# timmeinhardt/trackformer

Measured on AMD Instinct MI355X. Metric: frames/sec, TrackFormer-Deformable inference (ResNet-50, 1333x800, 300 object + 100 track queries, bs 1 per GPU); roofline = ms_deform_attn HBM GB/s, higher is better.
Workload: dtype f32 (dense layers as the fp16 split product on MFMA: two fp16 pieces per activation, three per weight scaled per output channel -- 22 + 1 significand bits per operand, the one dropped product < 2^-22 --, three terms, f32 accumulate)

## Files before the change

include/tf_fused.h:

```cpp
#ifndef TF_FUSED_H_
#define TF_FUSED_H_

#include <stdint.h>

#ifdef __cplusplus
extern "C" {
#endif

int tf_bias_act_f32(float *x, const float *bias, const float *residual, int64_t n, int C, int relu,
                    void *stream);

int tf_add_layernorm_f32(const float *x, const float *res, const float *gamma, const float *beta,
                         float *out, int64_t rows, int C, float eps, void *stream);

int tf_box_refine_f32(const float *delta, const float *ref, float *out, int64_t rows, int ref_dim, float eps, void *stream);

int tf_postprocess_pack_f32(const float *logits, const float *boxes, float *out, int64_t Q, int C, float img_h, float img_w,
                            int clip, void *stream);

int tf_groupnorm_nhwc_f32(const float *x, const float *gamma, const float *beta, float *out, double *workspace, int N,
                          int HW, int C, int G, float eps, int64_t x_image_stride, int64_t out_image_stride, void *stream);
int tf_groupnorm_stats_nhwc_f32(const float *x, double *workspace, int N, int HW, int C, int G, int64_t x_image_stride, void *stream);
int tf_groupnorm_relu_nhwc_f32(const float *x, const float *gamma, const float *beta, float *out, double *workspace, int N,
                               int HW, int C, int G, float eps, int64_t x_image_stride, int64_t out_image_stride, void *stream);
// ... 43 lines not shown
int tf_linear_packed_f32(const float *x, const void *w_packed, const float *bias, const float *residual, float *y, int64_t M, int K,
                         int N, int relu, int terms, void *stream);

int64_t tf_linear_grad_stats_workspace_bytes(int64_t M, int C, int role, int with_colsum);
int tf_linear_grad_stats_f32(const float *a, float *scale2, float *colsum, void *workspace, int64_t workspace_bytes, int64_t M, int C,
                             int role, int terms, void *stream);
int64_t tf_linear_wgrad_workspace_bytes(int64_t M, int K, int N);
int tf_linear_wgrad_split_f32(const float *dy, const float *x, const float *dy_scale2, const float *x_scale2, float *dw, void *workspace,
                              int64_t workspace_bytes, int64_t M, int K, int N, int terms, void *stream);
int tf_linear_dgrad_packed_f32(const float *dy, const float *dy_scale2, const void *wt_packed, float *dx, int64_t M, int K, int N,
                               int terms, void *stream);

int tf_conv_packed_f32(const float *x, const void *w_packed, const float *bias, const float *residual, float *y, float *workspace,
                       int ksplit, int nimg, int hin, int win, int cin, int cout, int ks, int stride, int relu, int terms,
                       void *stream);

int tf_linear_res_ln_f32(const float *x, const void *w_packed, const float *bias, const float *residual, const float *ln_weight,
                         const float *ln_bias, float ln_eps, float *y, int64_t M, int K, int N, int terms, void *stream);

int tf_ffn_fused_f32(const float *x, const void *w1_packed, const float *b1, const void *w2_packed, const float *b2,
                     const float *residual, const float *ln_weight, const float *ln_bias, float ln_eps, float *y, int64_t M,
                     int d_model, int d_ffn, int terms, void *stream);

int tf_mha_core_f32(const float *q, const float *k, const float *v, float *out, const unsigned char *key_mask,
                    int N, int Lq, int Lk, int H, int D, int ldq, int ldk, int ldv, int ldo, float scale,
                    void *stream);

int tf_nms_host_f32(const float *boxes, const float *scores, int n, float iou_threshold, int64_t *keep, int *n_keep);

#ifdef __cplusplus
}
#endif
#endif
```

trackformer_amd/_cabi.py:

```python
import ctypes
import os

_PKG_DIR = os.path.dirname(os.path.abspath(__file__))
LIB_PATH = os.environ.get("TF_MSDA_LIB") or os.path.join(_PKG_DIR, "lib", "libtf_msda.so")

EXPORTED_SYMBOLS = (
    "tf_msda_abi_version",
    "tf_msda_strerror",
    "tf_msda_last_hip_error",
    "tf_msda_last_kernel",
    "tf_msda_set_tiled",
    "tf_msda_set_option",
    "tf_msda_debug_trace_buffer",
    "tf_msda_forward_fused_f32",
    "tf_msda_forward_f32",
    "tf_msda_forward_f64",
    "tf_msda_forward_f32_dshapes",
    "tf_msda_forward_f64_dshapes",
    "tf_msda_backward_f32",
    "tf_msda_backward_f64",
    "tf_msda_backward_f32_dshapes",
    "tf_msda_backward_f64_dshapes",
    "tf_msda_backward_det_workspace_bytes",
    "tf_msda_backward_det_f32",
# ... 16 lines not shown
    "tf_mask_label_map_f32",
    "tf_conv3x3_merge_packed_f32",
    "tf_groupnorm_stats_nhwc_f32",
    "tf_groupnorm_relu_conv3x3_c1_nhwc_f32",
    "tf_bias_relu_maxpool_f32",
    "tf_stem_conv7x7_f32",
    "tf_linear_split_f32",
    "tf_linear_split_res_f32",
    "tf_conv3x3_split_f32",
    "tf_conv3x3_splitk_f32",
    "tf_conv1x1_strided_split_f32",
    "tf_conv1x1_splitk_f32",
    "tf_linear_packed_bytes",
    "tf_linear_pack_weight_f32",
    "tf_linear_packed_f32",
    "tf_linear_grad_stats_workspace_bytes",
    "tf_linear_grad_stats_f32",
    "tf_linear_wgrad_workspace_bytes",
    "tf_linear_wgrad_split_f32",
    "tf_linear_dgrad_packed_f32",
    "tf_linear_split_add_f32",
    "tf_ffn_fused_f32",
    "tf_linear_res_ln_f32",
    "tf_conv_packed_f32",
    "tf_mha_core_f32",
    "tf_nms_host_f32",
)

ABI_VERSION = 6

_lib = None


class MSDAError(RuntimeError):
    """Raised when libtf_msda.so reports a non-zero status."""


def lib():
    global _lib
    if _lib is not None:
        return _lib
    if not os.path.exists(LIB_PATH):
        raise RuntimeError(
            "trackformer_amd: native library %s not found. Build it with "
            "`python -m trackformer_amd.build` (needs hipcc); there is no CPU fallback." % LIB_PATH)
    import torch
    L = ctypes.CDLL(LIB_PATH)
    vp, ci = ctypes.c_void_p, ctypes.c_int
    L.tf_msda_abi_version.restype = ci
    L.tf_msda_abi_version.argtypes = []
    L.tf_msda_strerror.restype = ctypes.c_char_p
    L.tf_msda_strerror.argtypes = [ci]
    L.tf_msda_last_hip_error.restype = ci
    L.tf_msda_last_hip_error.argtypes = []
# ... 58 lines not shown
    for fn in (L.tf_groupnorm_nhwc_f32, L.tf_groupnorm_relu_nhwc_f32):
        fn.restype = ci
        fn.argtypes = [vp, vp, vp, vp, vp, ci, ci, ci, ci, ctypes.c_float, ctypes.c_int64, ctypes.c_int64, vp]
    L.tf_linear_split_f32.restype = ci
    L.tf_linear_split_f32.argtypes = [vp, vp, vp, vp, vp, vp, vp, ctypes.c_int64, ci, ci, ci, vp]
    L.tf_linear_split_res_f32.restype = ci
    L.tf_linear_split_res_f32.argtypes = [vp, vp, vp, vp, vp, vp, vp, vp, ctypes.c_int64, ci, ci, ci, vp]
    L.tf_conv3x3_splitk_f32.restype = ci
    L.tf_conv3x3_splitk_f32.argtypes = [vp, vp, vp, vp, vp, vp, vp, vp, ci, ci, ci, ci, ci, ci, ci, ci, vp]
    L.tf_conv3x3_split_f32.restype = ci
    L.tf_conv3x3_split_f32.argtypes = [vp, vp, vp, vp, vp, vp, vp] + [ci] * 7 + [vp]
    L.tf_conv1x1_splitk_f32.restype = ci
    L.tf_conv1x1_splitk_f32.argtypes = [vp, vp, vp, vp, vp, vp, vp, vp, ci, ci, ci, ci, ci, ci, ci, ci, vp]
    L.tf_conv1x1_strided_split_f32.restype = ci
    L.tf_conv1x1_strided_split_f32.argtypes = [vp, vp, vp, vp, vp, vp, vp] + [ci] * 7 + [vp]
    L.tf_linear_packed_bytes.restype = ctypes.c_int64
    L.tf_linear_packed_bytes.argtypes = [ci, ci, ci]
    L.tf_linear_pack_weight_f32.restype = ci
    L.tf_linear_pack_weight_f32.argtypes = [vp, vp, ci, ci, ci, vp]
    L.tf_linear_res_ln_f32.restype = ci
    L.tf_linear_res_ln_f32.argtypes = [vp, vp, vp, vp, vp, vp, ctypes.c_float, vp, ctypes.c_int64, ci, ci, ci, vp]
    L.tf_ffn_fused_f32.restype = ci
    L.tf_ffn_fused_f32.argtypes = [vp, vp, vp, vp, vp, vp, vp, vp, ctypes.c_float, vp, ctypes.c_int64, ci, ci, ci, vp]
    L.tf_linear_split_add_f32.restype = ci
    L.tf_linear_split_add_f32.argtypes = [vp, vp, vp, vp, vp, vp, vp, vp, ctypes.c_int64, ci, ci, vp]
    L.tf_linear_packed_f32.restype = ci
    L.tf_linear_packed_f32.argtypes = [vp, vp, vp, vp, vp, ctypes.c_int64, ci, ci, ci, ci, vp]
    i64 = ctypes.c_int64
    L.tf_linear_grad_stats_workspace_bytes.restype = i64
    L.tf_linear_grad_stats_workspace_bytes.argtypes = [i64, ci, ci, ci]
    L.tf_linear_grad_stats_f32.restype = ci
    L.tf_linear_grad_stats_f32.argtypes = [vp, vp, vp, vp, i64, i64, ci, ci, ci, vp]
    L.tf_linear_wgrad_workspace_bytes.restype = i64
    L.tf_linear_wgrad_workspace_bytes.argtypes = [i64, ci, ci]
    L.tf_linear_wgrad_split_f32.restype = ci
    L.tf_linear_wgrad_split_f32.argtypes = [vp, vp, vp, vp, vp, vp, i64, i64, ci, ci, ci, vp]
    L.tf_linear_dgrad_packed_f32.restype = ci
    L.tf_linear_dgrad_packed_f32.argtypes = [vp, vp, vp, vp, i64, ci, ci, ci, vp]
    L.tf_conv_packed_f32.restype = ci
    L.tf_conv_packed_f32.argtypes = [vp, vp, vp, vp, vp, vp] + [ci] * 10 + [vp]
    L.tf_mha_core_f32.restype = ci
    L.tf_mha_core_f32.argtypes = [vp, vp, vp, vp, vp] + [ci] * 9 + [ctypes.c_float, vp]
    if L.tf_msda_abi_version() != ABI_VERSION:
        raise RuntimeError("libtf_msda.so ABI version %d != expected %d (rebuild)" %
                           (L.tf_msda_abi_version(), ABI_VERSION))
    _lib = L
# ... 10 lines not shown
```

trackformer_amd/build.py:

```python
import hashlib
import os
import shutil
import subprocess
import sys
from concurrent.futures import ThreadPoolExecutor

PKG_DIR = os.path.dirname(os.path.abspath(__file__))
REPO_DIR = os.path.dirname(PKG_DIR)
CSRC = os.path.join(PKG_DIR, "csrc")
LIB_DIR = os.path.join(PKG_DIR, "lib")
INCLUDE = os.path.join(REPO_DIR, "include")
GFX_ARCH = "gfx950"

_TARGETS = [
    ("libtf_msda.so", ["msda_hip.hip", "msda_pquad.hip", "fused_ops.hip", "linear_split.hip", "linear_stream.hip", "mha_core.hip", "ffn_fused.hip", "stem_conv.hip", "msda_host.cpp"], []),
]


def _hipcc():
    exe = shutil.which("hipcc") or "/opt/rocm/bin/hipcc"
    if not os.path.exists(exe):
        raise RuntimeError("hipcc not found (expected on PATH or at /opt/rocm/bin/hipcc)")
    return exe

# ... 37 lines not shown
        src_paths = [os.path.join(CSRC, s) for s in srcs]
        flags = ["--offload-arch=" + GFX_ARCH, "-O3", "-std=c++17", "-fPIC", "-I" + INCLUDE,
                 "-Wno-pass-failed"] + extra
        key = _key(src_paths + headers, flags)
        if not force and not _stale(out, key):
            continue
        obj_dir = os.path.join(LIB_DIR, "obj")
        os.makedirs(obj_dir, exist_ok=True)
        objs = [os.path.join(obj_dir, os.path.splitext(s)[0] + ".o") for s in srcs]
        with ThreadPoolExecutor(max_workers=len(srcs)) as pool:
            list(pool.map(lambda so: _run([_hipcc()] + flags + ["-c", so[0], "-o", so[1]], verbose),
                          zip(src_paths, objs)))
        _run([_hipcc(), "--offload-arch=" + GFX_ARCH, "-shared", "-fPIC", "-pthread"] + objs + ["-o", out], verbose)
        _stamp(out, key)
        built.append(out)
    built += _build_tools(force, verbose)
    return built


def _build_tools(force, verbose):
    out_dir = os.path.join(REPO_DIR, "tools", "bin")
    lib = os.path.join(LIB_DIR, "libtf_msda.so")
    built = []
    for name in ("msda_bench", "linear_bench", "ffn_bench"):
        src = os.path.join(REPO_DIR, "tools", name + ".cpp")
        if not os.path.exists(src):
            continue
        os.makedirs(out_dir, exist_ok=True)
        out = os.path.join(out_dir, name)
        flags = ["--offload-arch=" + GFX_ARCH, "-O2", "-std=c++17", "-I" + INCLUDE]
        headers = [os.path.join(INCLUDE, f) for f in os.listdir(INCLUDE) if f.endswith(".h")]
        key = _key([src] + headers, flags)
        if not force and not _stale(out, key) and os.path.getmtime(out) >= os.path.getmtime(lib):
            continue
        _run([_hipcc()] + flags + [src, "-L" + LIB_DIR, "-ltf_msda",
                                   "-Wl,-rpath,$ORIGIN/../../trackformer_amd/lib", "-o", out], verbose)
        _stamp(out, key)
        built.append(out)
    return built


if __name__ == "__main__":
    res = build_all(force="--force" in sys.argv, verbose=True)
    print("built:" if res else "up to date", *res)
```

trackformer_amd/csrc/ffn_fused.hip:

```cpp
#include <hip/hip_runtime.h>

#include <stdint.h>
#include <stdlib.h>

#include <atomic>
#include <type_traits>

#include "msda_common.h"
#include "split_product.h"
#include "tf_fused.h"
#include "tf_msda.h"

namespace {

template <int D>
struct Geo {
    static_assert(D == 256 || D == 288, "hidden sizes of the reference's configurations");
    static constexpr int NW = D == 256 ? 4 : 3;
    static constexpr int NT = NW * 64;
    static constexpr int TJ = D / 32 / NW;
    static constexpr int XS = D + 8;
    static constexpr int CH = NW * 32;
    static constexpr int HS = CH + 8;
    static constexpr int KQ1 = D / 16;
// ... 411 lines not shown
        if (dev >= 32 || !(raised[ln ? 1 : 0].load() & (1u << dev))) {
            if (hipFuncSetAttribute(fn, hipFuncAttributeMaxDynamicSharedMemorySize, (int)lds) != hipSuccess) return TF_MSDA_ERR_LAUNCH;
            if (dev < 32) raised[ln ? 1 : 0].fetch_or(1u << dev);
        }
    }
    const int blocks = (M + 32 * TI - 1) / (32 * TI);
    void *argv[] = {(void *)&x, (void *)&w, (void *)&b, (void *)&res, (void *)&gamma, (void *)&beta, (void *)&eps, (void *)&y, (void *)&M};
    return hipLaunchKernel(fn, dim3((unsigned)blocks), dim3(Geo<D>::NT), argv, lds, s) == hipSuccess ? TF_MSDA_OK : TF_MSDA_ERR_LAUNCH;
}

std::atomic<int> g_linln_ti{-1};
int linln_ti()
{
    int v = g_linln_ti.load(std::memory_order_relaxed);
    if (v < 0) {
        const char *e = getenv("TF_LINLN_TI");
        v = e ? atoi(e) : 0;
        if (v < 0 || v > 3) v = 0;
        g_linln_ti.store(v);
    }
    return v;
}

std::atomic<int> g_ffn_tail{-1};
std::atomic<int> g_ffn_ti{-1};
int ffn_ti()
{
    int v = g_ffn_ti.load(std::memory_order_relaxed);
    if (v < 0) {
        const char *e = getenv("TF_FFN_TI");
        v = e ? atoi(e) : 3;
        if (v < 1 || v > 3) v = 3;
        g_ffn_ti.store(v);
    }
    return v;
}

}

namespace tfm {
int ffn_tail_split()
{
    int v = g_ffn_tail.load(std::memory_order_relaxed);
    if (v < 0) {
        const char *e = getenv("TF_FFN_TAIL_SPLIT");
        v = (e && e[0] == '0') ? 0 : 1;
        g_ffn_tail.store(v);
    }
    return v;
}
int ffn_set_tail_split(int v)
{
    const int prev = ffn_tail_split();
    g_ffn_tail.store(v ? 1 : 0);
    return prev;
}
int ffn_set_ti(int v)
{
    const int prev = ffn_ti();
    g_ffn_ti.store(v >= 1 && v <= 3 ? v : 3);
    return prev;
}
int linln_set_ti(int v)
{
    const int prev = linln_ti();
    g_linln_ti.store(v >= 1 && v <= 3 ? v : 0);
    return prev;
}
}

namespace {

int ffn_num_cus()
{
    static const int n = [] {
        int dev = 0, cus = 256;
        if (hipGetDevice(&dev) == hipSuccess) {
            hipDeviceProp_t prop;
            if (hipGetDeviceProperties(&prop, dev) == hipSuccess && prop.multiProcessorCount > 0) cus = prop.multiProcessorCount;
        }
        return cus;
    }();
    return n;
}

// ... 39 lines not shown
    }
}

template <int D>
int dispatch_linln_scheme(int sp, const float *x, const u32x4 *w, const float *bias, const float *residual, const float *g, const float *b,
                          float eps, float *y, int M, hipStream_t s)
{
    switch (sp) {
    case 3: return dispatch_linln<3, D>(x, w, bias, residual, g, b, eps, y, M, s);
    default: return dispatch_linln<16, D>(x, w, bias, residual, g, b, eps, y, M, s);
    }
}

template <int D>
int dispatch_ffn_scheme(int sp, const float *x, const u32x4 *w1, const float *b1, const u32x4 *w2, const float *b2, const float *residual,
                        const float *g, const float *b, float eps, float *y, int M, int F, hipStream_t s)
{
    switch (sp) {
    case 3: return dispatch_ffn<3, D>(x, w1, b1, w2, b2, residual, g, b, eps, y, M, F, s);
    default: return dispatch_ffn<16, D>(x, w1, b1, w2, b2, residual, g, b, eps, y, M, F, s);
    }
}

}

extern "C" int tf_linear_res_ln_f32(const float *x, const void *w_packed, const float *bias, const float *residual,
                                    const float *ln_weight, const float *ln_bias, float ln_eps, float *y, int64_t M, int K, int N,
                                    int terms, void *stream)
{
    if (!x || !w_packed || !y) return TF_MSDA_ERR_NULL_POINTER;
    if ((ln_weight == nullptr) != (ln_bias == nullptr)) return TF_MSDA_ERR_NULL_POINTER;
    const int sp = split_scheme(terms);
    if (M <= 0 || K != N || (K != 256 && K != 288) || (M + 128) * (int64_t)K * 4 > 0xFFFFFFFFLL || sp == 0) return TF_MSDA_ERR_BAD_DIMS;
    uintptr_t al = reinterpret_cast<uintptr_t>(x) | reinterpret_cast<uintptr_t>(w_packed) | reinterpret_cast<uintptr_t>(y) |
                   reinterpret_cast<uintptr_t>(bias) | reinterpret_cast<uintptr_t>(residual) | reinterpret_cast<uintptr_t>(ln_weight) |
                   reinterpret_cast<uintptr_t>(ln_bias);
    if (al & 15) return TF_MSDA_ERR_BAD_DIMS;
    const u32x4 *w = static_cast<const u32x4 *>(w_packed);
    hipStream_t s = static_cast<hipStream_t>(stream);
    return K == 256 ? dispatch_linln_scheme<256>(sp, x, w, bias, residual, ln_weight, ln_bias, ln_eps, y, (int)M, s)
                    : dispatch_linln_scheme<288>(sp, x, w, bias, residual, ln_weight, ln_bias, ln_eps, y, (int)M, s);
}

extern "C" int tf_ffn_fused_f32(const float *x, const void *w1_packed, const float *b1, const void *w2_packed, const float *b2,
                                const float *residual, const float *ln_weight, const float *ln_bias, float ln_eps, float *y,
                                int64_t M, int d_model, int d_ffn, int terms, void *stream)
// ... 17 lines not shown
```

trackformer_amd/csrc/msda_common.h:

```cpp
#ifndef TF_MSDA_COMMON_H_
#define TF_MSDA_COMMON_H_

#include <hip/hip_runtime.h>

#include "tf_msda.h"

namespace tfm {

struct LevelTable {
    int H[TF_MSDA_MAX_LEVELS];
    int W[TF_MSDA_MAX_LEVELS];
    int start[TF_MSDA_MAX_LEVELS];
};

typedef unsigned int u32x4_t __attribute__((ext_vector_type(4)));
typedef float f32x4_t __attribute__((ext_vector_type(4)));
#ifndef TF_STORE_AUX
#define TF_STORE_AUX 0
#endif
constexpr int kStoreAux = TF_STORE_AUX;
template <typename V>
__device__ __forceinline__ void stream_store(V *p, V v)
{
    if constexpr (kStoreAux == 2) __builtin_nontemporal_store(v, p);
// ... 11 lines not shown
};

struct DirectArgs {
    const float *value;
    unsigned value_bytes;
    const float *loc, *attn;
    float *out;
    FusedArgs fa;
    int S, M, L, Lq;
    long long nlq;
};

void note_kernel(const char *name);

bool launch_pquad(bool fused, const DirectArgs &da, const LevelTable &lt, int N, int D, int P, hipStream_t stream,
                  hipError_t *err);
int pquad_set_option(const char *name, int value);
void pquad_set_trace(unsigned long long *device_buffer);

int ffn_set_ti(int v);
int ffn_tail_split();
int ffn_set_tail_split(int v);
int linln_set_ti(int v);
int linear_stream_set_ti(int v);
int conv_halo_set(int v);
int linear_dma_set(int v);
int wgrad_msplit_set(int v);
int mha_set_mfma(int v);

}

#endif
```

trackformer_amd/csrc/msda_hip.hip:

```cpp
#include <hip/hip_runtime.h>

#include <limits.h>
#include <stdint.h>
#include <stdio.h>
#include <stdlib.h>
#include <string.h>

#include <atomic>
#include <type_traits>

#include "tf_msda.h"
#include "msda_common.h"
#include "msda_quad_geom.h"

namespace {
using namespace tfm;

constexpr int kThreads = 256;
constexpr int kLdsChunkBudget = 48 * 1024;

constexpr int kLevelTableBytes = 3 * TF_MSDA_MAX_LEVELS * (int)sizeof(int);

template <typename T, int VEC>
struct alignas(sizeof(T) * VEC) Pack {
// ... 1975 lines not shown
}

void tf_msda_debug_trace_buffer(void *device_buffer)
{
    g_quad_trace.store(static_cast<unsigned long long *>(device_buffer));
    pquad_set_trace(static_cast<unsigned long long *>(device_buffer));
}

int tf_msda_set_option(const char *name, int value)
{
    if (!name) return INT_MIN;
    if (strcmp(name, "tiled") == 0) return tf_msda_set_tiled(value);
    quad_opts_init();
    for (int i = 0; i < kQoCount; ++i)
        if (strcmp(name, kQuadOptNames[i]) == 0) {
            const int prev = g_quad_opt[i].exchange(value);
            g_quad_epoch.fetch_add(1);
            return prev;
        }
    if (strcmp(name, "direct9") == 0) return g_direct9.exchange(value < 0 ? -1 : (value ? 1 : 0));
    if (strcmp(name, "ffn_ti") == 0) return ffn_set_ti(value);
    if (strcmp(name, "ffn_tail_split") == 0) return ffn_set_tail_split(value);
    if (strcmp(name, "linln_ti") == 0) return linln_set_ti(value);
    if (strcmp(name, "linear_stream_ti") == 0) return linear_stream_set_ti(value);
    if (strcmp(name, "conv_halo") == 0) return conv_halo_set(value);
    if (strcmp(name, "linear_dma") == 0) return linear_dma_set(value);
    if (strcmp(name, "mha_mfma") == 0) return mha_set_mfma(value);
    if (strcmp(name, "wgrad_msplit") == 0) return wgrad_msplit_set(value);
    if (strncmp(name, "pquad", 5) == 0) {
        const int prev = pquad_set_option(name, value);
        return prev == -1 ? INT_MIN : prev;
    }
    return INT_MIN;
}

int tf_msda_forward_fused_f32(const float *value, const int64_t *shapes_hw_host,
                              const float *ref_points, int ref_dim, const float *qproj, int ld,
                              int off_col, int logit_col, float *out, int N, int S, int M, int D,
                              int L, int Lq, int P, void *stream)
{
    return forward_fused_impl(value, shapes_hw_host, ref_points, ref_dim, qproj, ld, off_col,
                              logit_col, out, N, S, M, D, L, Lq, P, stream);
}

int tf_msda_forward_f32(const float *value, const int64_t *shapes_hw_host, const float *loc,
                        const float *attn, float *out, int N, int S, int M, int D, int L, int Lq,
// ... 127 lines not shown
```

trackformer_amd/deformable_transformer.py:

```python
import copy
import math

import torch
import torch.nn.functional as F
from torch import nn
from torch.nn.init import constant_, normal_, xavier_uniform_

from . import fused
from .msda import MSDeformAttn, attach_host_shapes
from .nested import inverse_sigmoid, is_all_valid


def _inference(module) -> bool:
    return (not module.training) and (not torch.is_grad_enabled())


def _ffn_hidden(linear, activation, x, inference):
    if inference and activation is F.relu and x.is_cuda and x.dtype == torch.float32:
        if fused.split_linear_enabled():
            y = fused.linear(x, linear.weight, linear.bias, relu=True)
            if y is not None:
                return y
        x2 = x.reshape(-1, x.shape[-1])
        y = torch._addmm_activation(linear.bias, x2, linear.weight.t(), use_gelu=False)
# ... 395 lines not shown
            qk = fused.linear(qk_in, w, b[:2 * E], rows=(0, 2 * E))
        if qk is None:
            qk = F.linear(qk_in, w[:2 * E], b[:2 * E])
        v = fused.linear(v_in, w, b[2 * E:], rows=(2 * E, 3 * E))
        if v is None:
            v = F.linear(v_in, w[2 * E:], b[2 * E:])
        o = fused.mha_core(qk, v, H, key_padding_mask)
        if o is not None:
            if residual_norm is not None and fused.linear_ln_fused_enabled():
                y = fused.linear_residual_norm(o, mha.out_proj, residual_norm[0], residual_norm[1])
                if y is not None:
                    return y, True
            return fused.module_linear(mha.out_proj, o, True), False
        qk = qk.view(n, lq, 2, H, E // H)
        v = v.view(n, lq, H, E // H)
        q, k = qk[:, :, 0].transpose(1, 2), qk[:, :, 1].transpose(1, 2)
        mask = None
        if key_padding_mask is not None:
            mask = ~key_padding_mask[:, None, None, :]
        o = F.scaled_dot_product_attention(q, k, v.transpose(1, 2), attn_mask=mask)
        return mha.out_proj(o.transpose(1, 2).reshape(n, lq, E)), False

    def forward(self, tgt, query_pos, reference_points, src, src_spatial_shapes,
                src_padding_mask=None, query_attn_mask=None, filler_key_mask=None):
        key_mask = query_attn_mask if query_attn_mask is not None else filler_key_mask
        if _inference(self) and tgt.is_cuda and self.self_attn.in_proj_weight is not None:
            if query_pos is not None and fused.pos_add_fused_enabled():
                tgt2, normed = self._self_attention_inference(tgt, tgt, key_mask, residual_norm=(tgt, self.norm2), qk_pos=query_pos)
            else:
                tgt2, normed = self._self_attention_inference(self.with_pos_embed(tgt, query_pos), tgt, key_mask,
                                                              residual_norm=(tgt, self.norm2))
        else:
            normed = False
            q = k = self.with_pos_embed(tgt, query_pos)
            tgt2 = self.self_attn(q.transpose(0, 1), k.transpose(0, 1), tgt.transpose(0, 1),
                                  key_padding_mask=key_mask)[0].transpose(0, 1)
        tgt = tgt2 if normed else fused.residual_norm(tgt, self.dropout2(tgt2), self.norm2, _inference(self))
        inf = _inference(self)
        cq, cq_pos = (tgt, query_pos) if (inf and query_pos is not None and fused.pos_add_fused_enabled()) \
            else (self.with_pos_embed(tgt, query_pos), None)
        if inf and fused.linear_ln_fused_enabled():
            tgt = self.cross_attn(cq, reference_points, src, src_spatial_shapes, src_padding_mask, query_attn_mask,
                                  residual_norm=(tgt, self.norm1), query_pos=cq_pos)
            return self.forward_ffn(tgt)
        tgt2 = self.cross_attn(cq, reference_points, src, src_spatial_shapes, src_padding_mask, query_attn_mask,
                               query_pos=cq_pos)
        tgt = fused.residual_norm(tgt, self.dropout1(tgt2), self.norm1, _inference(self))
        return self.forward_ffn(tgt)


class DeformableTransformerDecoder(nn.Module):
    def __init__(self, decoder_layer, num_layers, return_intermediate=False):
        super().__init__()
        self.layers = _get_clones(decoder_layer, num_layers)
        self.num_layers = num_layers
        self.return_intermediate = return_intermediate
        self.bbox_embed = None
        self.class_embed = None

    def forward(self, tgt, reference_points, src, src_spatial_shapes, src_valid_ratios,
                query_pos=None, src_padding_mask=None, query_attn_mask=None, filler_key_mask=None):
        output = tgt
        intermediate = []
        intermediate_reference_points = []
        unit = getattr(src_valid_ratios, "_tf_unit", False)
        for lid, layer in enumerate(self.layers):
            if unit:
                reference_points_input = reference_points[:, :, None].expand(-1, -1, src_valid_ratios.shape[1], -1)
            elif reference_points.shape[-1] == 4:
                reference_points_input = reference_points[:, :, None] \
                    * torch.cat([src_valid_ratios, src_valid_ratios], -1)[:, None]
            else:
                assert reference_points.shape[-1] == 2
                reference_points_input = reference_points[:, :, None] * src_valid_ratios[:, None]
            output = layer(output, query_pos, reference_points_input, src, src_spatial_shapes,
                           src_padding_mask, query_attn_mask, filler_key_mask)

            if self.bbox_embed is not None:
                tmp = self.bbox_embed[lid](output)
                fused_ref = (fused.box_refine(tmp, reference_points)
                             if not self.training and not torch.is_grad_enabled() and tmp.is_cuda else None)
                if fused_ref is not None:
                    new_reference_points = fused_ref
                elif reference_points.shape[-1] == 4:
                    new_reference_points = (tmp + inverse_sigmoid(reference_points)).sigmoid()
                else:
                    assert reference_points.shape[-1] == 2
                    new_reference_points = tmp
                    new_reference_points[..., :2] = tmp[..., :2] + inverse_sigmoid(reference_points)
                    new_reference_points = new_reference_points.sigmoid()
                reference_points = new_reference_points.detach()

            if self.return_intermediate:
                intermediate.append(output)
                intermediate_reference_points.append(reference_points)

        if self.return_intermediate:
            return torch.stack(intermediate), torch.stack(intermediate_reference_points)
        return output, reference_points
# ... 26 lines not shown
```

trackformer_amd/fused.py:

```python
import os
import threading

import torch
import torch.nn.functional as F

from . import _cabi


def _stream(device):
    return torch.cuda.current_stream(device).cuda_stream


def _param_ok(t, x):
    return (t.device == x.device and t.dtype == torch.float32 and t.is_contiguous()
            and t.data_ptr() % 16 == 0)


_weight_epoch = 0
_route_epoch = 0


def weight_epoch():
    return _weight_epoch

# ... 515 lines not shown
            return None
        N = rows[1] - rows[0]
    if x.shape[-1] != K or K % 32 or x.numel() == 0:
        return None
    if bias is not None and not (bias.dtype == torch.float32 and bias.is_contiguous() and bias.numel() == N
                                 and bias.device == x.device):
        return None
    a, b = x.reshape(-1, K), x2.reshape(-1, K)
    a = a if a.is_contiguous() else a.contiguous()
    b = b if b.is_contiguous() else b.contiguous()
    pieces = _split_weight(weight)
    if rows is not None:
        pieces = _rows_of(pieces, rows)
    hi, mid, lo, wsc = pieces
    if (a.data_ptr() | b.data_ptr() | hi.data_ptr() | mid.data_ptr() | _ptr(lo)) & 15:
        return None
    with torch.cuda.device(x.device):
        y = torch.empty((a.shape[0], N), dtype=torch.float32, device=x.device)
        rc = _cabi.lib().tf_linear_split_add_f32(a.data_ptr(), b.data_ptr(), hi.data_ptr(), mid.data_ptr(), _ptr(lo), _ptr(wsc),
                                                 0 if bias is None else bias.data_ptr(), y.data_ptr(), a.shape[0], K, N,
                                                 _stream(x.device))
    _cabi.check(rc, "tf_linear_split_add_f32")
    return y.view(*x.shape[:-1], N)


def conv3x3(x, w_taps, bias, relu, stride):
    if not (_split_linear and x.is_cuda and x.dtype == torch.float32 and x.dim() == 4
            and x.is_contiguous(memory_format=torch.channels_last) and w_taps.dtype == torch.float32
            and w_taps.dim() == 2 and w_taps.is_contiguous() and w_taps.device == x.device):
        return None
    n, cin, h, w = x.shape
    cout = w_taps.shape[0]
    ks = 3 if w_taps.shape[1] == 9 * cin else 1
    if w_taps.shape[1] != ks * ks * cin or cin % 32 or stride not in (1, 2) or x.numel() == 0:
        return None
    if bias is not None and not (bias.dtype == torch.float32 and bias.is_contiguous() and bias.numel() == cout
                                 and bias.device == x.device):
        return None
    pad = 1 if ks == 3 else 0
    ho, wo = (h + 2 * pad - ks) // stride + 1, (w + 2 * pad - ks) // stride + 1
    cin_ok = cin % 64 == 0 or (ks == 3 and stride == 1 and _conv_halo and cin % 32 == 0)
    stream_route = (_conv_stream and _conv_stream_wins(n * ho * wo, cout) and cin_ok and not (x.data_ptr() & 15)
                    and n * h * w * cin * 4 < 0xC0000000 and (n * ho * wo + 256) * cout * 4 < 0xC0000000)
    halo = ks == 3 and stride == 1 and _conv_halo and stream_route
    ksplit = _conv_ksplit(n * ho * wo, ks * ks * cin, cout, _HALO_KSPLIT_POLICY if halo else None)
    if ks == 1 and (ksplit < _CONV1X1_MIN_PIECES or not _conv1x1_splitk):
# ... 634 lines not shown
```

trackformer_amd/msda.py:

```python
import ctypes
import math

import torch
import torch.nn.functional as F
from torch import nn
from torch.autograd import Function
from torch.autograd.function import once_differentiable
from torch.nn.init import constant_, xavier_uniform_

from . import _cabi, fused

import os as _os

FUSED_INFERENCE = _os.environ.get("TF_MSDA_FUSED", "1") != "0"

_HOST_SHAPE_ATTR = "_tf_msda_host_shapes"
_shape_array_cache = {}


def attach_host_shapes(spatial_shapes, host_shapes):
    setattr(spatial_shapes, _HOST_SHAPE_ATTR, tuple((int(h), int(w)) for h, w in host_shapes))
    return spatial_shapes


# ... 356 lines not shown
        self.output_proj = nn.Linear(d_model, d_model)
        self._cat_proj = _CatProjection()
        self._reset_parameters()

    def _reset_parameters(self):
        with torch.no_grad():
            constant_(self.sampling_offsets.weight, 0.)
        dirs = [(a, b) for a in (-1, 0, 1) for b in (-1, 0, 1) if (a, b) != (0, 0)]
        if self.n_heads != len(dirs):
            raise ValueError("MSDeformAttn bias initialisation requires n_heads == 8")
        grid = torch.tensor(dirs, dtype=torch.float32).view(self.n_heads, 1, 1, 2)
        grid = grid.repeat(1, self.n_levels, self.n_points, 1)
        scale = torch.arange(1, self.n_points + 1, dtype=torch.float32).view(1, 1, -1, 1)
        with torch.no_grad():
            self.sampling_offsets.bias = nn.Parameter((grid * scale).reshape(-1))
            constant_(self.attention_weights.weight, 0.)
            constant_(self.attention_weights.bias, 0.)
            xavier_uniform_(self.value_proj.weight)
            constant_(self.value_proj.bias, 0.)
            xavier_uniform_(self.output_proj.weight)
            constant_(self.output_proj.bias, 0.)

    def forward(self, query, reference_points, input_flatten, input_spatial_shapes,
                input_padding_mask=None, query_attn_mask=None, residual_norm=None, query_pos=None):
        if residual_norm is not None:
            out = self._forward(query, reference_points, input_flatten, input_spatial_shapes, input_padding_mask,
                                query_attn_mask, residual_norm, query_pos)
            if isinstance(out, _Normed):
                return out.value
            return fused.residual_norm(residual_norm[0], out, residual_norm[1], True)
        return self._forward(query, reference_points, input_flatten, input_spatial_shapes, input_padding_mask, query_attn_mask,
                             None, query_pos)

    def _forward(self, query, reference_points, input_flatten, input_spatial_shapes, input_padding_mask, query_attn_mask,
                 residual_norm, query_pos=None):
        N, Len_q, _ = query.shape
        N, Len_in, _ = input_flatten.shape
        hs = _host_shapes_of(input_spatial_shapes)
        if hs is not None:
            if sum(h * w for h, w in hs) != Len_in:
                raise AssertionError("sum of H_l*W_l does not match the flattened input length")
        else:
            assert (input_spatial_shapes[:, 0] * input_spatial_shapes[:, 1]).sum() == Len_in

        M, L, P = self.n_heads, self.n_levels, self.n_points
        inference = not self.training and not torch.is_grad_enabled()
        value = fused.module_linear(self.value_proj, input_flatten, inference)
        if input_padding_mask is not None:
            value = value.masked_fill(input_padding_mask[..., None], float(0))
        value = value.view(N, Len_in, M, self.d_model // M)

        if (FUSED_INFERENCE and hs is not None and query_attn_mask is None and value.is_cuda
                and value.dtype == torch.float32 and not self.training
                and not torch.is_grad_enabled() and reference_points.shape[-1] in (2, 4)
                and (self.d_model // M) % 4 == 0 and P in (1, 2, 4, 8)):
            w, b = self._cat_proj.get(self)
            qproj = None
            if query_pos is not None:
                qproj = fused.linear_add(query, query_pos, w, b)
                if qproj is None:
                    query = query + query_pos
            if qproj is None:
                qproj = fused.linear(query, w, b) if fused.split_linear_enabled() else None
            if qproj is None:
                qproj = F.linear(query, w, b)
            output = ms_deform_attn_forward_fused(value, input_spatial_shapes, reference_points,
                                                  qproj, M, L, P)
            if residual_norm is not None:
                y = fused.linear_residual_norm(output, self.output_proj, residual_norm[0], residual_norm[1])
                if y is not None:
                    return _Normed(y)
            return fused.module_linear(self.output_proj, output, True)

        if query_pos is not None:
            query = query + query_pos
        if torch.is_grad_enabled() and fused_training_enabled():
            if (hs is not None and query_attn_mask is None and value.is_cuda and value.dtype == torch.float32
                    and query.is_cuda and query.dtype == torch.float32 and reference_points.is_cuda
                    and reference_points.dtype == torch.float32 and reference_points.shape[-1] in (2, 4)
                    and (self.d_model // M) % 4 == 0 and P in (1, 2, 4, 8) and M * L * P <= _FUSED_TRAIN_MAX_ROW_SAMPLES):
                _fused_train_counts["fused"] += 1
# ... 28 lines not shown
```

Baseline: 374.9.

## Batch multiple projections sharing one input into a grouped split-GEMM kernel

Adds a grouped linear kernel that stages each activation row tile once in LDS and runs several projection weight sets over it, with an optional fused add of a second input (query_pos). In the encoder, value_proj and the concatenated offset/attention projection are computed in one launch. In the decoder, all layers' value_proj over the shared memory tensor are computed up front in batches of up to eight. This is meant to cut repeated activation reads and per-layer launch overhead, in exchange for extra LDS for the bias and scale tables, a larger and more complex kernel, and the memory to hold all decoder value tensors at once.

```diff
diff --git a/include/tf_fused.h b/include/tf_fused.h
--- a/include/tf_fused.h
+++ b/include/tf_fused.h
@@ -89,6 +89,16 @@
                      const float *residual, const float *ln_weight, const float *ln_bias, float ln_eps, float *y, int64_t M,
                      int d_model, int d_ffn, int terms, void *stream);
 
+typedef struct tf_proj_group {
+    const void *w_packed;
+    const float *bias;
+    float *y;
+    int N;
+    int add_x2;
+} tf_proj_group;
+int tf_linear_groups_f32(const float *x, const float *x2, const tf_proj_group *groups, int ngroups, int64_t M, int K, int terms,
+                         void *stream);
+
 int tf_mha_core_f32(const float *q, const float *k, const float *v, float *out, const unsigned char *key_mask,
                     int N, int Lq, int Lk, int H, int D, int ldq, int ldk, int ldv, int ldo, float scale,
                     void *stream);
diff --git a/trackformer_amd/_cabi.py b/trackformer_amd/_cabi.py
--- a/trackformer_amd/_cabi.py
+++ b/trackformer_amd/_cabi.py
@@ -62,6 +62,7 @@
     "tf_linear_split_add_f32",
     "tf_ffn_fused_f32",
     "tf_linear_res_ln_f32",
+    "tf_linear_groups_f32",
     "tf_conv_packed_f32",
     "tf_mha_core_f32",
     "tf_nms_host_f32",
@@ -70,6 +71,11 @@
 ABI_VERSION = 6
 
 _lib = None
+
+
+class ProjGroup(ctypes.Structure):
+    _fields_ = [("w_packed", ctypes.c_void_p), ("bias", ctypes.c_void_p), ("y", ctypes.c_void_p), ("N", ctypes.c_int),
+                ("add_x2", ctypes.c_int)]
 
 
 class MSDAError(RuntimeError):
@@ -174,6 +180,8 @@
     L.tf_linear_res_ln_f32.argtypes = [vp, vp, vp, vp, vp, vp, ctypes.c_float, vp, ctypes.c_int64, ci, ci, ci, vp]
     L.tf_ffn_fused_f32.restype = ci
     L.tf_ffn_fused_f32.argtypes = [vp, vp, vp, vp, vp, vp, vp, vp, ctypes.c_float, vp, ctypes.c_int64, ci, ci, ci, vp]
+    L.tf_linear_groups_f32.restype = ci
+    L.tf_linear_groups_f32.argtypes = [vp, vp, ctypes.POINTER(ProjGroup), ci, ctypes.c_int64, ci, ci, vp]
     L.tf_linear_split_add_f32.restype = ci
     L.tf_linear_split_add_f32.argtypes = [vp, vp, vp, vp, vp, vp, vp, vp, ctypes.c_int64, ci, ci, vp]
     L.tf_linear_packed_f32.restype = ci
diff --git a/trackformer_amd/build.py b/trackformer_amd/build.py
--- a/trackformer_amd/build.py
+++ b/trackformer_amd/build.py
@@ -83,7 +83,7 @@
     out_dir = os.path.join(REPO_DIR, "tools", "bin")
     lib = os.path.join(LIB_DIR, "libtf_msda.so")
     built = []
-    for name in ("msda_bench", "linear_bench", "ffn_bench"):
+    for name in ("msda_bench", "linear_bench", "ffn_bench", "proj_groups_bench"):
         src = os.path.join(REPO_DIR, "tools", name + ".cpp")
         if not os.path.exists(src):
             continue
diff --git a/trackformer_amd/csrc/ffn_fused.hip b/trackformer_amd/csrc/ffn_fused.hip
--- a/trackformer_amd/csrc/ffn_fused.hip
+++ b/trackformer_amd/csrc/ffn_fused.hip
@@ -457,6 +457,7 @@
     return v;
 }
 
+std::atomic<int> g_groups_ti{0};
 std::atomic<int> g_ffn_tail{-1};
 std::atomic<int> g_ffn_ti{-1};
 int ffn_ti()
@@ -496,6 +497,7 @@
     g_ffn_ti.store(v >= 1 && v <= 3 ? v : 3);
     return prev;
 }
+int groups_set_ti(int v) { return g_groups_ti.exchange(v >= 1 && v <= 3 ? v : 0); }
 int linln_set_ti(int v)
 {
     const int prev = linln_ti();
@@ -581,6 +583,263 @@
     }
 }
 
+constexpr int kMaxProjGroups = 8;
+struct ProjGroup {
+    const u32x4 *w;
+    const float *bias;
+    float *y;
+    int N, cbase;
+};
+struct ProjGroups {
+    ProjGroup g[kMaxProjGroups];
+    int ng, nplain;
+    int ncols;
+    int nchunk[2][2];
+    int chunk[32];
+};
+constexpr int kMaxProjCols = 4096;
+struct ChunkW {
+    const u32x4 *base;
+    int us, as;
+    bool half;
+};
+
+template <int SP, int TI, bool ADD>
+__device__ __forceinline__ void stage_rows_sum(const __amdgpu_buffer_rsrc_t xrs, const __amdgpu_buffer_rsrc_t x2rs, int m0, unsigned short *sX, int tid)
+{
+    using G = Geo<256>;
+    constexpr int D = 256, C4 = D / 4, NV = TI * 32 * C4 / G::NT, RPI = G::NT / C4;
+    static_assert(G::NT % C4 == 0, "a pass of the block covers whole rows");
+    const int row0 = tid / C4, c4 = tid - row0 * C4;
+    const unsigned voff = (unsigned)((m0 + row0) * D + c4 * 4) * 4u;
+    f32x4 xr[NV], xr2[ADD ? NV : 1];
+#pragma unroll
+    for (int it = 0; it < NV; ++it) {
+        xr[it] = __builtin_bit_cast(f32x4, __builtin_amdgcn_raw_buffer_load_b128(xrs, voff, (unsigned)(it * RPI * D * 4), 0));
+        if constexpr (ADD) xr2[it] = __builtin_bit_cast(f32x4, __builtin_amdgcn_raw_buffer_load_b128(x2rs, voff, (unsigned)(it * RPI * D * 4), 0));
+    }
+    __builtin_amdgcn_sched_barrier(0);
+#pragma unroll
+    for (int it = 0; it < NV; ++it) {
+        f32x4 xv = xr[it];
+        if constexpr (ADD) xv += xr2[it];
+        u32x2 pc[Split<SP>::NA];
+        split4<SP>(xv, pc);
+#pragma unroll
+        for (int p = 0; p < Split<SP>::NA; ++p) *reinterpret_cast<u32x2 *>(&sX[(p * TI * 32 + it * RPI + row0) * G::XS + c4 * 4]) = pc[p];
+    }
+}
+
+template <int SP, int TI>
+__global__ void __launch_bounds__(256, (linln_min_blocks(256, TI)))
+linear_groups_kernel(const float *__restrict__ X, const float *__restrict__ X2, int M, const ProjGroups pg)
+{
+    using G = Geo<256>;
+    constexpr int BM = TI * 32, XS = G::XS, KQ = G::KQ1, NA = Split<SP>::NA, NB = Split<SP>::NB, US = 2 * NB;
+    constexpr bool F16 = Split<SP>::F16;
+    constexpr int RING = linln_ring(TI), AHEAD = RING - 2;
+    static_assert(KQ % RING == 0 && (KQ / 2) % RING == 0 && AHEAD <= KQ / 2, "a chunk starts at ring slot 0");
+    extern __shared__ __attribute__((aligned(16))) unsigned short s_f[];
+    unsigned short *const sX = s_f;
+    float *const sBias = reinterpret_cast<float *>(s_f + NA * BM * XS);
+    float *const sScale = sBias + pg.ncols;
+    const int tid = threadIdx.x, lane = tid & 63;
+    const int wave = __builtin_amdgcn_readfirstlane(tid >> 6);
+    const int m0 = blockIdx.x * BM;
+    const int frow = lane & 31, xoff = frow * XS + (lane >> 5) * 8;
+
+    auto chunk_of = [&](int code) {
+        const ProjGroup &g = pg.g[code >> 16];
+        const int col0 = (code & 0x7fff) * 128;
+        ChunkW c;
+        c.half = (code >> 15) & 1;
+        const int tile = (col0 >> 5) + (c.half ? wave : 2 * wave);
+        c.base = g.w + (size_t)tile * (KQ * NB * 64) + lane;
+        c.us = c.half ? 2 * NB : NB;
+        c.as = c.half ? NB : KQ * NB;
+        return c;
+    };
+    u32x4 ring[RING][US];
+    auto load_unit = [&](const ChunkW &c, auto uc, u32x4 (&dst)[US]) {
+        constexpr int u = decltype(uc)::value;
+        const u32x4 *p0 = c.base + (size_t)(u * c.us) * 64;
+#pragma unroll
+        for (int a = 0; a < 2; ++a)
+#pragma unroll
+            for (int p = 0; p < NB; ++p) dst[a * NB + p] = p0[(size_t)(a * c.as + p) * 64];
+    };
+    u32x4 xf[2][TI][NA];
+    auto read_x = [&](auto stc) {
+        constexpr int st = decltype(stc)::value;
+#pragma unroll
+        for (int i = 0; i < TI; ++i)
+#pragma unroll
+            for (int p = 0; p < NA; ++p)
+                xf[st & 1][i][p] = *reinterpret_cast<const u32x4 *>(&sX[(p * BM + i * 32) * XS + xoff + st * 16]);
+    };
+
+    auto run_chunk = [&](auto halfc, const ChunkW &cur, const ChunkW &nxt, int code) {
+        constexpr bool HALF = decltype(halfc)::value;
+        constexpr int TJ = HALF ? 1 : 2, UNITS = HALF ? KQ / 2 : KQ;
+        const ProjGroup &g = pg.g[code >> 16];
+        const int col0 = (code & 0x7fff) * 128;
+        const int N = g.N;
+        const int wcol = col0 + wave * (32 * TJ);
+        f32x16 acc[TI][TJ];
+#pragma unroll
+        for (int i = 0; i < TI; ++i)
+#pragma unroll
+            for (int j = 0; j < TJ; ++j)
+#pragma unroll
+                for (int e = 0; e < 16; ++e) acc[i][j][e] = 0.f;
+        read_x(std::integral_constant<int, 0>{});
+        static_for<KQ>([&](auto stc) {
+            constexpr int st = decltype(stc)::value;
+            constexpr int u = HALF ? st / 2 : st;
+            if constexpr (!HALF || (st & 1) == 0) {
+                constexpr int ahead = u + AHEAD;
+                if constexpr (ahead < UNITS) load_unit(cur, std::integral_constant<int, ahead>{}, ring[ahead % RING]);
+                else load_unit(nxt, std::integral_constant<int, ahead - UNITS>{}, ring[ahead % RING]);
+            }
+            if constexpr (st + 1 < KQ) read_x(std::integral_constant<int, st + 1>{});
+            __builtin_amdgcn_sched_barrier(0);
+            const u32x4 (&cu)[US] = ring[u % RING];
+            u32x4 wf[TJ][NB];
+#pragma unroll
+            for (int j = 0; j < TJ; ++j)
+#pragma unroll
+                for (int p = 0; p < NB; ++p) wf[j][p] = cu[(HALF ? (st & 1) : j) * NB + p];
+            mfma_tiles<SP, TI, TJ, false>(acc, xf[st & 1], wf);
+        });
+        const unsigned ybytes = (unsigned)((size_t)M * N * 4);
+#pragma unroll
+        for (int j = 0; j < TJ; ++j) {
+            const __amdgpu_buffer_rsrc_t yrs = __builtin_amdgcn_make_buffer_rsrc(g.y, 0, wcol + 32 * j < N ? ybytes : 0u, 0x00020000);
+#pragma unroll
+            for (int q = 0; q < 4; ++q) {
+                const int col = wcol + 32 * j + 8 * q + 4 * (lane >> 5);
+                const f32x4 bv = *reinterpret_cast<const f32x4 *>(sBias + g.cbase + col);
+                f32x4 rv = {1.f, 1.f, 1.f, 1.f};
+                if constexpr (F16) rv = *reinterpret_cast<const f32x4 *>(sScale + g.cbase + col);
+#pragma unroll
+                for (int i = 0; i < TI; ++i) {
+                    f32x4 v;
+#pragma unroll
+                    for (int e = 0; e < 4; ++e) v[e] = F16 ? __builtin_fmaf(acc[i][j][4 * q + e], rv[e], bv[e]) : acc[i][j][4 * q + e] + bv[e];
+                    __builtin_amdgcn_raw_buffer_store_b128(__builtin_bit_cast(u32x4, v), yrs,
+                                                           (unsigned)((m0 + i * 32 + frow) * N + col) * 4u, 0, tfm::kStoreAux);
+                }
+            }
+        }
+    };
+
+    const int total = pg.nchunk[0][0] + pg.nchunk[0][1] + pg.nchunk[1][0] + pg.nchunk[1][1];
+    int ci = 0;
+    ChunkW cur = chunk_of(pg.chunk[0]);
+    static_for<AHEAD>([&](auto uc) { load_unit(cur, uc, ring[decltype(uc)::value]); });
+    __builtin_amdgcn_sched_barrier(0);
+    const unsigned xbytes = (unsigned)((size_t)M * 256 * 4);
+    const __amdgpu_buffer_rsrc_t xrs = __builtin_amdgcn_make_buffer_rsrc(const_cast<float *>(X), 0, xbytes, 0x00020000);
+    const __amdgpu_buffer_rsrc_t x2rs = __builtin_amdgcn_make_buffer_rsrc(const_cast<float *>(X2 ? X2 : X), 0, xbytes, 0x00020000);
+    for (int gq = 0; gq < pg.ng; ++gq) {
+        const ProjGroup &g = pg.g[gq];
+        const int npad = (g.N + 255) / 256 * 256;
+        const float *const r = reinterpret_cast<const float *>(g.w + (size_t)(npad / 32) * KQ * NB * 64);
+        const __amdgpu_buffer_rsrc_t brs =
+            __builtin_amdgcn_make_buffer_rsrc(const_cast<float *>(g.bias ? g.bias : X), 0, g.bias ? (unsigned)g.N * 4u : 0u, 0x00020000);
+        for (int c = tid * 4; c < npad; c += 4 * G::NT) {
+            *reinterpret_cast<f32x4 *>(sBias + g.cbase + c) = __builtin_bit_cast(f32x4, __builtin_amdgcn_raw_buffer_load_b128(brs, (unsigned)c * 4u, 0, 0));
+            if constexpr (F16) *reinterpret_cast<f32x4 *>(sScale + g.cbase + c) = *reinterpret_cast<const f32x4 *>(r + c);
+        }
+    }
+    if (pg.nplain == 0) stage_rows_sum<SP, TI, true>(xrs, x2rs, m0, sX, tid);
+    else stage_rows_sum<SP, TI, false>(xrs, x2rs, m0, sX, tid);
+    __syncthreads();
+#pragma unroll 1
+    for (int ph = 0; ph < 2; ++ph) {
+        if (ph == 1 && pg.nplain > 0 && pg.nplain < pg.ng) {
+            __syncthreads();
+            stage_rows_sum<SP, TI, true>(xrs, x2rs, m0, sX, tid);
+            __syncthreads();
+        }
+#pragma unroll 1
+        for (int k = 0; k < pg.nchunk[ph][0]; ++k, ++ci) {
+            const ChunkW nxt = chunk_of(pg.chunk[min(ci + 1, total - 1)]);
+            run_chunk(std::false_type{}, cur, nxt, pg.chunk[ci]);
+            cur = nxt;
+        }
+#pragma unroll 1
+        for (int k = 0; k < pg.nchunk[ph][1]; ++k, ++ci) {
+            const ChunkW nxt = chunk_of(pg.chunk[min(ci + 1, total - 1)]);
+            run_chunk(std::true_type{}, cur, nxt, pg.chunk[ci]);
+            cur = nxt;
+        }
+    }
+}
+
+template <int SP, int TI>
+int launch_groups(const float *x, const float *x2, int M, const ProjGroups &pg, hipStream_t s)
+{
+    constexpr size_t tile = linln_lds_bytes<256>(TI, Split<SP>::NA), lds_max = tile + 2 * 4 * kMaxProjCols;
+    static_assert(lds_max <= 160 * 1024, "the activation tile and the tables do not fit the LDS of a CU");
+    const size_t lds = tile + 2 * 4 * (size_t)pg.ncols;
+    const void *fn = (const void *)&linear_groups_kernel<SP, TI>;
+    if (lds_max > 64 * 1024) {
+        static std::atomic<unsigned> raised;
+        int dev = 0;
+        (void)hipGetDevice(&dev);
+        if (dev >= 32 || !(raised.load() & (1u << dev))) {
+            if (hipFuncSetAttribute(fn, hipFuncAttributeMaxDynamicSharedMemorySize, (int)lds_max) != hipSuccess) return TF_MSDA_ERR_LAUNCH;
+            if (dev < 32) raised.fetch_or(1u << dev);
+        }
+    }
+    const int blocks = (M + 32 * TI - 1) / (32 * TI);
+    void *argv[] = {(void *)&x, (void *)&x2, (void *)&M, (void *)&pg};
+    return hipLaunchKernel(fn, dim3((unsigned)blocks), dim3(256), argv, lds, s) == hipSuccess ? TF_MSDA_OK : TF_MSDA_ERR_LAUNCH;
+}
+
+}
+
+extern "C" int tf_linear_groups_f32(const float *x, const float *x2, const tf_proj_group *groups, int ngroups, int64_t M, int K, int terms,
+                                    void *stream)
+{
+    if (!x || !groups) return TF_MSDA_ERR_NULL_POINTER;
+    if (ngroups < 1 || ngroups > kMaxProjGroups) return TF_MSDA_ERR_BAD_DIMS;
+    for (int i = 0; i < ngroups; ++i)
+        if (!groups[i].w_packed || !groups[i].y || (groups[i].add_x2 && !x2)) return TF_MSDA_ERR_NULL_POINTER;
+    const int sp = split_scheme(terms);
+    if (M <= 0 || K != 256 || sp == 0 || (M + 128) * (int64_t)K * 4 > 0xFFFFFFFFLL) return TF_MSDA_ERR_BAD_DIMS;
+    uintptr_t al = reinterpret_cast<uintptr_t>(x) | reinterpret_cast<uintptr_t>(x2);
+    ProjGroups pg{};
+    for (int pass = 0; pass < 2; ++pass)
+        for (int i = 0; i < ngroups; ++i) {
+            const tf_proj_group &g = groups[i];
+            if ((g.add_x2 != 0) != (pass == 1)) continue;
+            if (g.N <= 0 || (g.N % 32) != 0 || (M + 128) * (int64_t)g.N * 4 > 0xFFFFFFFFLL) return TF_MSDA_ERR_BAD_DIMS;
+            al |= reinterpret_cast<uintptr_t>(g.w_packed) | reinterpret_cast<uintptr_t>(g.bias) | reinterpret_cast<uintptr_t>(g.y);
+            pg.g[pg.ng++] = ProjGroup{static_cast<const u32x4 *>(g.w_packed), g.bias, g.y, g.N, pg.ncols};
+            pg.ncols += (g.N + 255) / 256 * 256;
+            if (pass == 0) pg.nplain = pg.ng;
+        }
+    if ((al & 15) || pg.ncols > kMaxProjCols) return TF_MSDA_ERR_BAD_DIMS;
+    int nc = 0;
+    for (int ph = 0; ph < 2; ++ph)
+        for (int half = 0; half < 2; ++half)
+            for (int gi = ph ? pg.nplain : 0; gi < (ph ? pg.ng : pg.nplain); ++gi) {
+                const int N = pg.g[gi].N, full_end = N / 256 * 256;
+                for (int col0 = half ? full_end : 0; col0 < (half ? N : full_end); col0 += half ? 128 : 256) {
+                    pg.chunk[nc++] = gi << 16 | half << 15 | col0 / 128;
+                    ++pg.nchunk[ph][half];
+                }
+            }
+    hipStream_t s = static_cast<hipStream_t>(stream);
+    if (sp == 3) return launch_groups<3, 1>(x, x2, (int)M, pg, s);
+    const int forced = g_groups_ti.load(std::memory_order_relaxed);
+    switch (forced ? forced : (M < 4096 ? 1 : 3)) {
+    case 1: return launch_groups<16, 1>(x, x2, (int)M, pg, s);
+    case 2: return launch_groups<16, 2>(x, x2, (int)M, pg, s);
+    default: return launch_groups<16, 3>(x, x2, (int)M, pg, s);
+    }
 }
 
 extern "C" int tf_linear_res_ln_f32(const float *x, const void *w_packed, const float *bias, const float *residual,
diff --git a/trackformer_amd/csrc/msda_common.h b/trackformer_amd/csrc/msda_common.h
--- a/trackformer_amd/csrc/msda_common.h
+++ b/trackformer_amd/csrc/msda_common.h
@@ -57,6 +57,7 @@
 int ffn_tail_split();
 int ffn_set_tail_split(int v);
 int linln_set_ti(int v);
+int groups_set_ti(int v);
 int linear_stream_set_ti(int v);
 int conv_halo_set(int v);
 int linear_dma_set(int v);
diff --git a/trackformer_amd/csrc/msda_hip.hip b/trackformer_amd/csrc/msda_hip.hip
--- a/trackformer_amd/csrc/msda_hip.hip
+++ b/trackformer_amd/csrc/msda_hip.hip
@@ -2021,6 +2021,7 @@
     if (strcmp(name, "ffn_ti") == 0) return ffn_set_ti(value);
     if (strcmp(name, "ffn_tail_split") == 0) return ffn_set_tail_split(value);
     if (strcmp(name, "linln_ti") == 0) return linln_set_ti(value);
+    if (strcmp(name, "groups_ti") == 0) return groups_set_ti(value);
     if (strcmp(name, "linear_stream_ti") == 0) return linear_stream_set_ti(value);
     if (strcmp(name, "conv_halo") == 0) return conv_halo_set(value);
     if (strcmp(name, "linear_dma") == 0) return linear_dma_set(value);
diff --git a/trackformer_amd/deformable_transformer.py b/trackformer_amd/deformable_transformer.py
--- a/trackformer_amd/deformable_transformer.py
+++ b/trackformer_amd/deformable_transformer.py
@@ -441,7 +441,7 @@
         return mha.out_proj(o.transpose(1, 2).reshape(n, lq, E)), False
 
     def forward(self, tgt, query_pos, reference_points, src, src_spatial_shapes,
-                src_padding_mask=None, query_attn_mask=None, filler_key_mask=None):
+                src_padding_mask=None, query_attn_mask=None, filler_key_mask=None, src_value=None):
         key_mask = query_attn_mask if query_attn_mask is not None else filler_key_mask
         if _inference(self) and tgt.is_cuda and self.self_attn.in_proj_weight is not None:
             if query_pos is not None and fused.pos_add_fused_enabled():
@@ -460,10 +460,10 @@
             else (self.with_pos_embed(tgt, query_pos), None)
         if inf and fused.linear_ln_fused_enabled():
             tgt = self.cross_attn(cq, reference_points, src, src_spatial_shapes, src_padding_mask, query_attn_mask,
-                                  residual_norm=(tgt, self.norm1), query_pos=cq_pos)
+                                  residual_norm=(tgt, self.norm1), query_pos=cq_pos, value=src_value)
             return self.forward_ffn(tgt)
         tgt2 = self.cross_attn(cq, reference_points, src, src_spatial_shapes, src_padding_mask, query_attn_mask,
-                               query_pos=cq_pos)
+                               query_pos=cq_pos, value=src_value)
         tgt = fused.residual_norm(tgt, self.dropout1(tgt2), self.norm1, _inference(self))
         return self.forward_ffn(tgt)
 
@@ -483,6 +483,14 @@
         intermediate = []
         intermediate_reference_points = []
         unit = getattr(src_valid_ratios, "_tf_unit", False)
+        src_values = [None] * len(self.layers)
+        if (fused.proj_groups_enabled("dec") and src.is_cuda and not torch.is_grad_enabled()
+                and all(_inference(layer) and _inference(layer.cross_attn) for layer in self.layers)):
+            for a in range(0, len(self.layers), 8):
+                projs = [layer.cross_attn.value_proj for layer in self.layers[a:a + 8]]
+                ys = fused.linear_groups(src, None, [(p.weight, p.bias, False) for p in projs])
+                if ys is not None:
+                    src_values[a:a + len(ys)] = ys
         for lid, layer in enumerate(self.layers):
             if unit:
                 reference_points_input = reference_points[:, :, None].expand(-1, -1, src_valid_ratios.shape[1], -1)
@@ -493,7 +501,7 @@
                 assert reference_points.shape[-1] == 2
                 reference_points_input = reference_points[:, :, None] * src_valid_ratios[:, None]
             output = layer(output, query_pos, reference_points_input, src, src_spatial_shapes,
-                           src_padding_mask, query_attn_mask, filler_key_mask)
+                           src_padding_mask, query_attn_mask, filler_key_mask, src_value=src_values[lid])
 
             if self.bbox_embed is not None:
                 tmp = self.bbox_embed[lid](output)
diff --git a/trackformer_amd/fused.py b/trackformer_amd/fused.py
--- a/trackformer_amd/fused.py
+++ b/trackformer_amd/fused.py
@@ -561,6 +561,90 @@
                                                  _stream(x.device))
     _cabi.check(rc, "tf_linear_split_add_f32")
     return y.view(*x.shape[:-1], N)
+
+
+def _parse_proj_groups(v):
+    v = str(v).strip().lower()
+    if v in ("", "0", "off", "false"):
+        return frozenset()
+    if v in ("1", "on", "true", "all"):
+        return frozenset(("enc", "dec"))
+    routes = frozenset(t.strip() for t in v.split(",") if t.strip())
+    if not routes <= {"enc", "dec"}:
+        raise ValueError("TF_PROJ_GROUPS: 0, 1 or a comma-separated subset of enc,dec")
+    return routes
+
+
+_PROJ_GROUPS_DEFAULT = "enc,dec"
+_proj_groups = _parse_proj_groups(os.environ.get("TF_PROJ_GROUPS", _PROJ_GROUPS_DEFAULT))
+_PROJ_GROUPS_MIN_ROWS = int(os.environ.get("TF_PROJ_GROUPS_MIN_ROWS", "4096"))
+
+
+def proj_groups_enabled(route=None):
+    return bool(_proj_groups) if route is None else route in _proj_groups
+
+
+def set_proj_groups(on):
+    global _proj_groups
+    if isinstance(on, (set, frozenset, list, tuple)):
+        new = _parse_proj_groups(",".join(sorted(on)))
+    elif isinstance(on, str):
+        new = _parse_proj_groups(on)
+    else:
+        new = _parse_proj_groups("1" if on else "0")
+    prev, _proj_groups = _proj_groups, new
+    return _switched(prev, _proj_groups)
+
+
+def set_proj_groups_min_rows(n):
+    global _PROJ_GROUPS_MIN_ROWS
+    prev, _PROJ_GROUPS_MIN_ROWS = _PROJ_GROUPS_MIN_ROWS, int(n)
+    return _switched(prev, _PROJ_GROUPS_MIN_ROWS)
+
+
+def linear_groups(x, x2, groups):
+    if not (_split_linear and x.is_cuda and x.dtype == torch.float32 and 1 <= len(groups) <= 8 and x.numel()):
+        return None
+    if _split_terms == 16 and (_n_six_term_routes or debug_checks_active()):
+        return None
+    K = x.shape[-1]
+    if K != 256:
+        return None
+    any_add = any(add for _w, _b, add in groups)
+    if any_add and (x2 is None or x2.dtype != torch.float32 or x2.shape != x.shape or x2.device != x.device):
+        return None
+    a = x.reshape(-1, K)
+    a = a if a.is_contiguous() else a.contiguous()
+    M = a.shape[0]
+    if M < _PROJ_GROUPS_MIN_ROWS or (M + 128) * K * 4 > 0xFFFFFFFF:
+        return None
+    b = None
+    if any_add:
+        b = x2.reshape(-1, K)
+        b = b if b.is_contiguous() else b.contiguous()
+    if (a.data_ptr() | _ptr(b)) & 15:
+        return None
+    cols = 0
+    for w, bias, _add in groups:
+        if not (w.dtype == torch.float32 and w.dim() == 2 and w.is_contiguous() and w.device == x.device and w.shape[1] == K
+                and w.shape[0] % 32 == 0 and (M + 128) * w.shape[0] * 4 <= 0xFFFFFFFF):
+            return None
+        if bias is not None and not (_param_ok(bias, x) and bias.numel() == w.shape[0]):
+            return None
+        cols += (w.shape[0] + 255) // 256 * 256
+    if cols > 4096:
+        return None
+    packed = [_packed_weight(w, None) for w, _b, _add in groups]
+    if any(p is None for p in packed):
+        return None
+    descs = (_cabi.ProjGroup * len(groups))()
+    with torch.cuda.device(x.device):
+        ys = [torch.empty((M, w.shape[0]), dtype=torch.float32, device=x.device) for w, _b, _add in groups]
+        for d, (w, bias, add), p, y in zip(descs, groups, packed, ys):
+            d.w_packed, d.bias, d.y, d.N, d.add_x2 = p.data_ptr(), (bias.data_ptr() if bias is not None else None), y.data_ptr(), w.shape[0], int(bool(add))
+        rc = _cabi.lib().tf_linear_groups_f32(a.data_ptr(), _ptr(b) or None, descs, len(groups), M, K, _terms(), _stream(x.device))
+    _cabi.check(rc, "tf_linear_groups_f32")
+    return [y.view(*x.shape[:-1], y.shape[1]) for y in ys]
 
 
 def conv3x3(x, w_taps, bias, relu, stride):
diff --git a/trackformer_amd/msda.py b/trackformer_amd/msda.py
--- a/trackformer_amd/msda.py
+++ b/trackformer_amd/msda.py
@@ -402,18 +402,18 @@
             constant_(self.output_proj.bias, 0.)
 
     def forward(self, query, reference_points, input_flatten, input_spatial_shapes,
-                input_padding_mask=None, query_attn_mask=None, residual_norm=None, query_pos=None):
+                input_padding_mask=None, query_attn_mask=None, residual_norm=None, query_pos=None, value=None):
         if residual_norm is not None:
             out = self._forward(query, reference_points, input_flatten, input_spatial_shapes, input_padding_mask,
-                                query_attn_mask, residual_norm, query_pos)
+                                query_attn_mask, residual_norm, query_pos, value)
             if isinstance(out, _Normed):
                 return out.value
             return fused.residual_norm(residual_norm[0], out, residual_norm[1], True)
         return self._forward(query, reference_points, input_flatten, input_spatial_shapes, input_padding_mask, query_attn_mask,
-                             None, query_pos)
+                             None, query_pos, value)
 
     def _forward(self, query, reference_points, input_flatten, input_spatial_shapes, input_padding_mask, query_attn_mask,
-                 residual_norm, query_pos=None):
+                 residual_norm, query_pos=None, value=None):
         N, Len_q, _ = query.shape
         N, Len_in, _ = input_flatten.shape
         hs = _host_shapes_of(input_spatial_shapes)
@@ -425,18 +425,26 @@
 
         M, L, P = self.n_heads, self.n_levels, self.n_points
         inference = not self.training and not torch.is_grad_enabled()
-        value = fused.module_linear(self.value_proj, input_flatten, inference)
+        fused_inference = (FUSED_INFERENCE and hs is not None and query_attn_mask is None and inference
+                           and reference_points.shape[-1] in (2, 4) and (self.d_model // M) % 4 == 0 and P in (1, 2, 4, 8))
+        qproj = None
+        if value is not None and not inference:
+            raise ValueError("MSDeformAttn: a precomputed `value` is an inference-path extension")
+        if (value is None and fused_inference and query_pos is not None and input_flatten is query and fused.proj_groups_enabled("enc")
+                and fused.pos_add_fused_enabled()):
+            w, b = self._cat_proj.get(self)
+            ys = fused.linear_groups(query, query_pos, [(self.value_proj.weight, self.value_proj.bias, False), (w, b, True)])
+            if ys is not None:
+                value, qproj = ys
+        if value is None:
+            value = fused.module_linear(self.value_proj, input_flatten, inference)
         if input_padding_mask is not None:
             value = value.masked_fill(input_padding_mask[..., None], float(0))
         value = value.view(N, Len_in, M, self.d_model // M)
 
-        if (FUSED_INFERENCE and hs is not None and query_attn_mask is None and value.is_cuda
-                and value.dtype == torch.float32 and not self.training
-                and not torch.is_grad_enabled() and reference_points.shape[-1] in (2, 4)
-                and (self.d_model // M) % 4 == 0 and P in (1, 2, 4, 8)):
+        if fused_inference and value.is_cuda and value.dtype == torch.float32:
             w, b = self._cat_proj.get(self)
-            qproj = None
-            if query_pos is not None:
+            if qproj is None and query_pos is not None:
                 qproj = fused.linear_add(query, query_pos, w, b)
                 if qproj is None:
                     query = query + query_pos
```

Result: faster. 381.4 (median of 6 runs) (+1.7%).
